# granne/granne

Measured on AMD Instinct MI355X. Metric: queries/sec (recall@10 alongside), 10M x 100-d angular, batch=1024, higher is better.
Workload: dtype f32; 1 GPU; C2 (BASELINE.json configs[1]): 10000000 x 100-d f32 angular, i.i.d. uniform components, batch=1024, ef_search=50, k=10; n_elements=10000000, dim=100, batch=1024, ef_search=50, k=10

## Files before the change

granne_amd/_lib.py:

```python
import ctypes as C
import os

from . import build as _build

F32, I8, F16 = 0, 1, 2
UNUSED = 0xFFFFFFFF
BUILD_ALL = 0xFFFFFFFFFFFFFFFF

OK = 0
ERR_INVALID, ERR_HIP, ERR_NO_DEVICE, ERR_OVERFLOW, ERR_IO = -1, -2, -3, -4, -5

OPT_VISITED_SLOTS, OPT_FORCE_SLOW, OPT_SLOW_SLOTS, OPT_SLOW_BLOCKS, OPT_OVERFLOW_SLOTS = 1, 2, 3, 4, 5
OPT_VISITED16, OPT_VISITED16_LG, OPT_LAST_WALKER, OPT_SEARCH_DEPTH, OPT_INLINE_TAILS, OPT_SEEN_MIN = 6, 7, 8, 9, 10, 11
OPT_SKETCH = 12
OPT_COALESCE, OPT_COALESCE_MAX, OPT_COALESCE_WAIT_US, OPT_COALESCED_LAUNCHES, OPT_COALESCED_QUERIES = 13, 14, 15, 16, 17
OPT_LAST_COMPACT_ROWS = 18
OPT_LAST_SPLIT_TAIL = 19
OPT_LAST_SCAN = 20
OPT_FORCE_GENERAL = 21
(SCAN_NONE, SCAN_RING, SCAN_I8, SCAN_I8_CHUNKED, SCAN_B16_7_4, SCAN_B16_13_2, SCAN_B16_16_1, SCAN_B16_CHUNKED, SCAN_F32_52_4,
 SCAN_F32_100_2, SCAN_F32_128_1) = range(11)
EXACT_TOPK_KMAX = 1024
EXACT_TOPK_CAP = 4096
PF_MAX_STAGES = 8
# ... 54 lines not shown
    "granne_hip_index_create": (i32, [C.POINTER(vp), vp, u64, u32, i32, u32, vp, vp, vp, i32]),
    "granne_hip_index_create_csr": (i32, [C.POINTER(vp), vp, u64, u32, i32, u32, vp, vp, vp, i32]),
    "granne_hip_index_create_device": (i32, [C.POINTER(vp), vp, u64, u32, i32, u32, vp, vp, vp, i32, vp]),
    "granne_hip_index_destroy": (None, [vp]),
    "granne_hip_index_len": (u64, [vp]),
    "granne_hip_index_num_elements": (u64, [vp]),
    "granne_hip_index_num_layers": (u32, [vp]),
    "granne_hip_index_layer_len": (u64, [vp, u32]),
    "granne_hip_index_dim": (u32, [vp]),
    "granne_hip_index_dtype": (i32, [vp]),
    "granne_hip_index_device": (i32, [vp]),
    "granne_hip_index_hbm_bytes": (u64, [vp]),
    "granne_hip_index_get_neighbors": (i32, [vp, u64, u32, vp, u32, C.POINTER(u32)]),
    "granne_hip_index_get_element": (i32, [vp, u64, vp]),
    "granne_hip_index_get_sketch": (i32, [vp, u64, u64, vp]),
    "granne_hip_search_batch": (i32, [vp, vp, u32, u32, u32, vp, vp, vp, vp]),
    "granne_hip_search_batch_device": (i32, [vp, vp, u32, u32, u32, vp, vp, vp, vp, vp, vp]),
    "granne_hip_search_batches_device": (i32, [vp, u32, vp, u32, u32, u32, vp, vp, vp, vp, vp, vp]),
    "granne_hip_search_begin_device": (i32, [vp, vp, u32, u32, u32, vp, vp, vp, vp, vp, vp, C.POINTER(u64)]),
    "granne_hip_search_end_device": (i32, [vp, u64, vp]),
    "granne_hip_device_malloc": (i32, [C.POINTER(vp), u64, i32]),
    "granne_hip_device_free": (i32, [vp, i32]),
    "granne_hip_copy_to_device": (i32, [vp, vp, u64, i32, vp]),
    "granne_hip_copy_to_host": (i32, [vp, vp, u64, i32, vp]),
    "granne_hip_stream_create": (i32, [C.POINTER(vp), i32]),
    "granne_hip_stream_destroy": (i32, [vp, i32]),
    "granne_hip_stream_synchronize": (i32, [vp, i32]),
    "granne_hip_event_create": (i32, [vp]),
    "granne_hip_event_destroy": (None, [vp]),
    "granne_hip_event_elapsed_ms": (i32, [vp, vp, vp]),
# ... 171 lines not shown
```

granne_amd/csrc/granne_hip.hip:

```cpp
#include <hip/hip_runtime.h>

#include <atomic>
#include <chrono>
#include <cstdarg>
#include <cstdio>
#include <cstdlib>
#include <cstring>
#include <memory>
#include <mutex>
#include <string>
#include <type_traits>
#include <vector>

#include "../../include/granne_hip.h"
#include "search_kernel.h"
#include "walk_fast.h"
#include "slow_kernel.h"
#include "util_kernels.h"
#include "brute_force.h"
#include "exact_topk.h"
#include "combiner.h"
#include "dev_mem.h"

using namespace granne_hip;
// ... 339 lines not shown
    const size_t bytes = (size_t)n * SKETCH_LINE;
    if (!ix->d_sketch) {
        size_t free_b = 0, total_b = 0;
        if (hipMemGetInfo(&free_b, &total_b) != hipSuccess) {
            (void)hipGetLastError();
            return GRANNE_HIP_OK;
        }
        if ((uint64_t)free_b < (uint64_t)bytes + total_b / 32u) return GRANNE_HIP_OK;
        if (ix->d_sketch.alloc(bytes) != hipSuccess) {
            (void)hipGetLastError();
            return GRANNE_HIP_OK;
        }
        ix->hbm_bytes += bytes;
    }
    hipLaunchKernelGGL(row_sketch_kernel, dim3(grid_for(n, 256)), dim3(256), 0, s, ix->d_elements.as<uint8_t>(), n, ix->row_stride, ix->dim,
                       ix->d_sketch.as<uint8_t>());
    HIP_TRY(hipGetLastError());
    return GRANNE_HIP_OK;
}

static int finish_layers(granne_hip_index* ix, hipStream_t s) {
    std::vector<LayerDev> h(ix->layers.size());
    ix->max_dev_width = 32;
    {
        int r = make_inline_tails(ix, s);
        if (r == 0) r = make_scan_norms(ix, s);
        if (r == 0) r = make_row_sketch(ix, s);
        if (r) return r;
    }
    DevBuf found_buf;
    std::vector<uint32_t> found(h.size(), 0u);
// ... 214 lines not shown
    *out_count = n;
    for (uint32_t i = 0; i < n && i < cap && out_ids; ++i) out_ids[i] = row[i];
    return GRANNE_HIP_OK;
}

extern "C" int granne_hip_index_get_element(const granne_hip_index* ix, uint64_t idx, void* out) {
    if (!ix || !out) return fail(GRANNE_HIP_ERR_INVALID, "null argument");
    if (idx >= ix->n_elements) return fail(GRANNE_HIP_ERR_INVALID, "element index out of range");
    if (ix->se) return se_rows_to_host(*ix->se, idx, 1, 1, (float*)out);
    DeviceGuard g(ix->device);
    HIP_TRY(hipMemcpy(out, ix->d_elements.as<uint8_t>() + idx * ix->row_stride, (size_t)ix->dim * elem_size(ix->dtype),
                      hipMemcpyDeviceToHost));
    return GRANNE_HIP_OK;
}

extern "C" int granne_hip_index_get_sketch(const granne_hip_index* ix, uint64_t first, uint64_t count, void* out) {
    if (!ix || (!out && count)) return fail(GRANNE_HIP_ERR_INVALID, "null argument");
    GRANNE_HIP_COMPACT_UNSUPPORTED(ix, "get_sketch");
    if (!ix->d_sketch) return fail(GRANNE_HIP_ERR_INVALID, "the index holds no row sketches");
    if (first > ix->n_elements || count > ix->n_elements - first) return fail(GRANNE_HIP_ERR_INVALID, "rows out of range");
    if (count == 0) return GRANNE_HIP_OK;
    DeviceGuard g(ix->device);
    HIP_TRY(hipMemcpy(out, ix->d_sketch.as<uint8_t>() + first * SKETCH_LINE, (size_t)count * SKETCH_LINE, hipMemcpyDeviceToHost));
    return GRANNE_HIP_OK;
}

extern "C" int granne_hip_index_set_option(granne_hip_index* ix, int option, uint64_t value) {
    if (!ix) return fail(GRANNE_HIP_ERR_INVALID, "index is null");
    switch (option) {
    case GRANNE_HIP_OPT_VISITED_SLOTS:
        {
            const uint64_t odd = value ? value >> __builtin_ctzll(value) : 1;
            if (value != 0 && (value < 256 || value > 32768 || (odd != 1 && odd != 3)))
                return fail(GRANNE_HIP_ERR_INVALID, "visited slots must be 0, 2^k or 3 * 2^k in [256, 32768]");
        }
// ... 387 lines not shown
    const int vmode = T.opt_visited16 ? (int)T.opt_visited16 : knobs().visited;
    const bool none = vmode == 4 || vmode == 0;
    const bool longest = walk_list_is_long((int)P.S, wide) || wide;
    uint32_t walk_lds;
    if (fast && !trail && ((none && !T.opt_visited_slots) || longest)) {
        const uint32_t touch_max = knobs().touch_max >= 0 ? (uint32_t)knobs().touch_max : 256u;
        const bool touch_shape = P.S == 1 && !wide && !streamed && !(i8 && T.stage_row_bytes != 128);
        P.v16 = (touch_shape && nq <= touch_max) ? 4 : 3;
        const uint64_t seen_min = knobs().seen_min >= 0 ? (uint64_t)knobs().seen_min : T.opt_seen_min;
        if (P.S <= 4 && !wide && !i8 && nq >= seen_min) P.v16 = 5;
        P.cr = P.v16 == 5 && !i8 && sketch_dim_ok(T.dim) && T.d_sketch != nullptr && knobs().compact_rows != 0;
        P.split = P.cr && !wide;
        walk_lds = fast_lds_bytes(i8, streamed, T.dim, T.stage_row_bytes, P.S, 0u, P.v16 == 5, wide);
        const uint32_t least = lds_query_bytes(T.stage_row_bytes) + 64u * 8u;
        if (walk_lds < least) walk_lds = least;
    } else {
        uint32_t want = T.opt_visited_slots ? (uint32_t)T.opt_visited_slots : next_pow2(ef_walk * 64u);
        if (!T.opt_visited_slots) {
            if (want < 1024) want = 1024;
            uint32_t cap = nq >= 4096 ? 4096u : 8192u;
            if (fast && P.S >= 8) cap = 4096u;
            if (want > cap) want = cap;
        }
        P.visited_slots = want;
        P.upper_slots = want < 1024 ? want : 1024;
        if (fast) {
            walk_lds = fast_lds_bytes(i8, streamed, T.dim, T.stage_row_bytes, P.S, P.visited_slots, false, wide);
        } else {
            P.adjspec_bytes = i8 ? 0u : LDS_ADJSPEC_BYTES;
            const uint32_t fixed = lds_query_bytes(T.stage_row_bytes) + LDS_FIXED_BYTES + P.adjspec_bytes;
// ... 1171 lines not shown
```

granne_amd/csrc/search_kernel.h:

```cpp
#pragma once

#include "dist.h"
#include "wave_prims.h"
#include "sum_embeddings.h"
#include "f16.h"
#include "filter.h"

namespace granne_hip {

constexpr int DT_F32 = 0;
constexpr int DT_I8 = 1;

struct LayerDev {
    const uint32_t* adj;
    uint64_t len;
    uint32_t width;
    uint32_t flags;
    const uint8_t* adjx;
    uint32_t adjx_stride;
    uint32_t reserved;
};
constexpr uint32_t LAYER_TWIN_ROWS = 1u;

constexpr uint32_t SKETCH_LINE = 128u;
constexpr uint32_t SKETCH_META = 112u;
constexpr uint32_t SKETCH_MAX_DIM = 112u;
__host__ __device__ constexpr bool sketch_dim_ok(uint32_t dim) { return dim == 100u; }

constexpr uint32_t MAX_LAUNCH_BATCHES = 32;
struct BatchIO {
    const uint8_t* queries;
    uint64_t* out_ids;
    float* out_dists;
    uint32_t* out_counts;
    uint64_t* out_stats;
};

struct SearchParams {
    const uint8_t* elements;
    uint64_t n_elements;
// ... 629 lines not shown
```

granne_amd/csrc/util_kernels.h:

```cpp
#pragma once

#include "dist.h"
#include "ordered_sum.h"
#include "search_kernel.h"

namespace granne_hip {

__device__ __forceinline__ float sketch_ceil_sqrt(double S) {
    const double T = S * (1.0 + 0x1p-40);
    if (!(T <= (double)3.4028234663852886e38 * (double)3.4028234663852886e38)) return __builtin_inff();
    float f = (float)__builtin_sqrt(T);
    while ((double)f * (double)f < T) f = __uint_as_float(__float_as_uint(f) + 1u);
    while (f > 0.0f) {
        const float g = __uint_as_float(__float_as_uint(f) - 1u);
        if ((double)g * (double)g < T) break;
        f = g;
    }
    return f;
}

__global__ void row_sketch_kernel(const uint8_t* __restrict__ elements, uint64_t n, uint32_t row_stride, uint32_t dim,
                                  uint8_t* __restrict__ out) {
    for (uint64_t row = (uint64_t)blockIdx.x * blockDim.x + threadIdx.x; row < n; row += (uint64_t)gridDim.x * blockDim.x) {
        const float* x = reinterpret_cast<const float*>(elements + row * row_stride);
        uint32_t* o = reinterpret_cast<uint32_t*>(out + row * SKETCH_LINE);
        float m = 0.0f;
        bool finite = true;
        for (uint32_t i = 0; i < dim; ++i) {
            const float a = __builtin_fabsf(x[i]);
            finite = finite && a <= 3.4028234663852886e38f;
            m = a > m ? a : m;
        }
        const float s = finite ? (float)((double)m / 127.0) : 0.0f;
        double se = 0.0, sc = 0.0, sx = 0.0;
        for (uint32_t j = 0; j < SKETCH_META / 4u; ++j) {
            uint32_t w = 0;
            for (uint32_t t = 0; t < 4u; ++t) {
// ... 2 lines not shown
                const double xd = (double)x[i];
                double c = 0.0;
                if (s > 0.0f) {
                    c = __builtin_rint(xd / (double)s);
                    c = c < -127.0 ? -127.0 : (c > 127.0 ? 127.0 : c);
                }
                const double pc = (double)s * c, e = xd - pc;
                se = se + e * e;
                sc = sc + pc * pc;
                sx = sx + xd * xd;
                w |= ((uint32_t)(int32_t)c & 0xFFu) << (8u * t);
            }
            o[j] = w;
        }
        const float inf = __builtin_inff();
        o[SKETCH_META / 4u + 0u] = __float_as_uint(s);
        o[SKETCH_META / 4u + 1u] = __float_as_uint(finite ? sketch_ceil_sqrt(se) : inf);
        o[SKETCH_META / 4u + 2u] = __float_as_uint(finite ? sketch_ceil_sqrt(sc) : inf);
        o[SKETCH_META / 4u + 3u] = __float_as_uint(finite ? sketch_ceil_sqrt(sx) : inf);
    }
}

__global__ void relayout_rows_kernel(const uint8_t* __restrict__ src, uint8_t* __restrict__ dst, uint64_t n,
                                     uint32_t src_bytes, uint32_t dst_bytes) {
    const uint32_t units = dst_bytes >> 4;
    uint64_t total = n * units;
    for (uint64_t t = (uint64_t)blockIdx.x * blockDim.x + threadIdx.x; t < total;
         t += (uint64_t)gridDim.x * blockDim.x) {
        uint64_t row = t / units;
        uint32_t u = (uint32_t)(t - row * units);
        const uint8_t* s = src + row * src_bytes + (uint64_t)u * 16;
        uint32_t avail = (u * 16 < src_bytes) ? min(16u, src_bytes - u * 16) : 0u;
        uint32_t w[4] = {0, 0, 0, 0};
        uint8_t* wb = reinterpret_cast<uint8_t*>(w);
// ... 385 lines not shown
```

granne_amd/csrc/walk_fast.h:

```cpp
#pragma once

#include <type_traits>

#include "slow_kernel.h"

namespace granne_hip {

#ifndef GRANNE_HIP_PHASE_TIMERS
#define GRANNE_HIP_PHASE_TIMERS 0
#endif
#if GRANNE_HIP_PHASE_TIMERS
constexpr uint32_t PHASE_SLOTS = 48, PHASE_QUERIES = 4096;
__device__ uint64_t g_phase[PHASE_QUERIES * PHASE_SLOTS];
#define PT_MARK(i)                                                                   \
    do {                                                                             \
        asm volatile("" ::: "memory");                                               \
        __builtin_amdgcn_sched_barrier(0);                                           \
        const uint64_t now_ = __builtin_amdgcn_s_memtime();                          \
        const uint64_t dt_ = now_ - pt_last;                                         \
        if (pt_bottom) pt_b[i] += dt_; else pt_u[i] += dt_;                          \
        pt_last = now_;                                                              \
        __builtin_amdgcn_sched_barrier(0);                                           \
        asm volatile("" ::: "memory");                                               \
    } while (0)
// ... 14 lines not shown
#define PT_COUNT() do {} while (0)
#define PT_PIN(v) do {} while (0)
#define PT_ADD(i, n) do {} while (0)
#endif

__device__ __forceinline__ uint64_t wkey(float d, uint32_t id) {
    return ((uint64_t)__float_as_uint(d) << 32) | ((uint64_t)id << 1);
}
__device__ __forceinline__ uint32_t wkey_hi(uint64_t k) { return (uint32_t)(k >> 32); }
__device__ __forceinline__ uint32_t wkey_id(uint64_t k) { return ((uint32_t)k) >> 1; }
__device__ __forceinline__ float wkey_dist(uint64_t k) { return __uint_as_float((uint32_t)(k >> 32)); }
constexpr uint32_t WPOS_NONE = 0xFFFFFFFFu;
constexpr uint32_t VCACHE_SLOTS = 512;
constexpr uint32_t VCACHE_SLOTS_SEEN = 2048;
constexpr uint64_t WALK_MAX_ELEMENTS = 1ull << 31;
#ifndef GRANNE_HIP_CR_G
#define GRANNE_HIP_CR_G 8
#endif
#ifndef GRANNE_HIP_CR_WAVES
#define GRANNE_HIP_CR_WAVES 0
#endif
static_assert(GRANNE_HIP_CR_G == 8 || GRANNE_HIP_CR_G == 4, "a surviving row is held by 8 or by 4 lanes");
static_assert(GRANNE_HIP_CR_WAVES == 0 || (GRANNE_HIP_CR_WAVES >= 4 && GRANNE_HIP_CR_WAVES <= 6), "the table's value, or four to six waves per SIMD");
__host__ __device__ constexpr int cr_waves(int S) {
    return GRANNE_HIP_CR_WAVES ? GRANNE_HIP_CR_WAVES : S == 1 ? 6 : 5;
}
__host__ __device__ constexpr uint32_t fast_vcache_slots(bool seen, bool sketched, int S) {
    return seen ? ((sketched && cr_waves(S) >= 5) ? 1024u : VCACHE_SLOTS_SEEN) : VCACHE_SLOTS;
}

// ... 306 lines not shown
            } else {
#pragma unroll
                for (int u = 0; u < TU; ++u) rr.vt[u] = *reinterpret_cast<const float4*>(row + NB * 128 + u * 16);
            }
        } else {
            const uint8_t* e = p.elements + (size_t)idl * RSTRIDE + h * 64u;
#pragma unroll
            for (int b = 0; b < NBI; ++b)
#pragma unroll
                for (int k = 0; k < 4; ++k) rr.x[b * 4 + k] = *reinterpret_cast<const uint4*>(e + b * 128 + k * 16);
        }
        asm volatile("" ::: "memory");
    }

    __device__ __forceinline__ uint64_t sketch_rejects(const uint32_t nb, const bool go, RowRegs& rr) {
        if (go) {
            const uint8_t* line = p.sketch + (size_t)nb * SKETCH_LINE + h * 64u;
#pragma unroll
            for (int k = 0; k < 4; ++k) rr.v[0][k] = *reinterpret_cast<const float4*>(line + k * 16);
        }
        asm volatile("" ::: "memory");
        int ip = 0;
#pragma unroll
        for (int k = 0; k < 4; ++k) {
            const uint4 qq = *reinterpret_cast<const uint4*>(sk_qc + h * 64u + k * 16);
            ip = dot4_i8(__float_as_uint(rr.v[0][k].x), qq.x, ip);
            ip = dot4_i8(__float_as_uint(rr.v[0][k].y), qq.y, ip);
            ip = dot4_i8(__float_as_uint(rr.v[0][k].z), qq.z, ip);
            ip = dot4_i8(__float_as_uint(rr.v[0][k].w), qq.w, ip);
        }
        ip += pair_swap(ip);
        static_assert(SKETCH_META == 64u + 48u, "s, R, X, N: the last 16 bytes of the odd lane's half");
        const float sx = rr.v[0][3].x, rx = rr.v[0][3].y, xx = rr.v[0][3].z, nx = rr.v[0][3].w;
        const float t = (sk_s * sx) * (float)ip;
        const float nqnx = sk_n * nx;
        const float b = (sk_r * xx + sk_n * rx) + nqnx * 0x1p-17f;
        const float U = t + ((__builtin_fabsf(t) * 0x1p-20f + b * 1.0001f) + 0x1p-20f);
        const float lb = 1.0f - U;
        const uint64_t rm = wave_ballot(go && h != 0u && nqnx < 0x1p100f && lb > __uint_as_float(theta));
        return rm | (rm >> 1);
    }

    __device__ __forceinline__ float finish_rows(RowRegs& rr) {
        float d;
        if constexpr (GEN) {
            float acc[16];
#pragma unroll
            for (int j = 0; j < 16; ++j) acc[j] = 0.0f;
// ... 89 lines not shown
            if (q != q) q = 0.0f;
            const float t = 1.0f - q;
            d = (0.0f <= t) ? t : 0.0f;
        }
        return d;
    }

    static constexpr int CG = CR ? CR : 8;
    static constexpr int CU = 8 / CG;
    static constexpr uint32_t CNG = 64u / CG;
    struct CRows {
        float4 v[NB ? NB : 1][CU];
        float4 vt[TU ? TU : 1];
    };
    __device__ __forceinline__ uint64_t* cr_slots() const { return mslot + CAP; }
    __device__ __forceinline__ void cr_issue(CRows& c, const uint64_t e, const bool act, const uint32_t ct, const uint8_t* xtails) const {
        if (act) {
            const uint8_t* row = p.elements + (size_t)(uint32_t)e * RSTRIDE;
#pragma unroll
            for (int b = 0; b < NB; ++b)
#pragma unroll
                for (int u = 0; u < CU; ++u) c.v[b][u] = *reinterpret_cast<const float4*>(row + b * 128 + (ct * CU + u) * 16u);
            const uint8_t* tp = xtails ? xtails + (uint32_t)(e >> 32) * XTAILB : row + NB * 128;
#pragma unroll
            for (int u = 0; u < TU; ++u) {
                const uint4 t = load_global_u4((gptr_u32)(tp + u * 16));
                c.vt[u] = make_float4(__uint_as_float(t.x), __uint_as_float(t.y), __uint_as_float(t.z), __uint_as_float(t.w));
            }
        }
    }
    __device__ __forceinline__ float cr_finish(const CRows& c, const uint32_t ct) const {
        typedef float f32x2 __attribute__((ext_vector_type(2)));
        f32x2 acc2[2 * CU];
#pragma unroll
        for (int j = 0; j < 2 * CU; ++j) acc2[j] = f32x2{0.0f, 0.0f};
#pragma unroll
        for (int b = 0; b < NB; ++b) {
#pragma unroll
            for (int u = 0; u < CU; ++u) {
                const float4 qq = *reinterpret_cast<const float4*>(lds_q + b * 128 + (ct * CU + u) * 16u);
                acc2[u * 2 + 0] = __builtin_elementwise_fma(f32x2{c.v[b][u].x, c.v[b][u].y}, f32x2{qq.x, qq.y}, acc2[u * 2 + 0]);
                acc2[u * 2 + 1] = __builtin_elementwise_fma(f32x2{c.v[b][u].z, c.v[b][u].w}, f32x2{qq.z, qq.w}, acc2[u * 2 + 1]);
// ... 11 lines not shown
            s = __uint_as_float((uint32_t)__builtin_amdgcn_update_dpp(0, __float_as_int(s), 0x111 , 0xf, 0xf, true) & keep);
#pragma unroll
            for (int j = 0; j < 4 * CU; ++j) s = s + acc[j];
        }
        float r = s;
#pragma unroll
        for (int u = 0; u < TU; ++u) {
            const float4 qq = *reinterpret_cast<const float4*>(lds_q + NB * 128 + u * 16);
            r = __builtin_fmaf(c.vt[u].x, qq.x, r);
            r = __builtin_fmaf(c.vt[u].y, qq.y, r);
            r = __builtin_fmaf(c.vt[u].z, qq.z, r);
            r = __builtin_fmaf(c.vt[u].w, qq.w, r);
        }
        return angular_from_dot(r);
    }
    __device__ __forceinline__ float compact_rows(const uint32_t ns, const uint32_t srank, const bool surv, const uint8_t* xtails) const {
        const uint32_t ct = lane & (uint32_t)(CG - 1), g = lane / (uint32_t)CG;
        const uint64_t* cs = cr_slots();
        float d = 0.0f;
        uint32_t base = 0;
        CRows ra;
#pragma unroll 1
        do {
            const uint32_t sa = base + g;
            const uint64_t ea = cs[sa];
            cr_issue(ra, ea, sa < ns, ct, xtails);
            asm volatile("" ::: "memory");
            const uint32_t rel = srank - base;
            const int from = (int)(((rel & (CNG - 1u)) * (uint32_t)CG + (uint32_t)(CG - 1)) * 4u);
            const float da = cr_finish(ra, ct);
            const float ba = __int_as_float(__builtin_amdgcn_ds_bpermute(from, __float_as_int(da)));
            d = (surv && rel < CNG) ? ba : d;
            base += CNG;
        } while (base < ns);
        return d;
    }

    static constexpr bool LONG = List::LONG;
    static constexpr int LONG_STEPS = CAP >= 4096u ? 7 : 6;
    static constexpr uint32_t FCAP = 63u;
    static constexpr uint32_t FIMG_KEYS = 128u;
// ... 521 lines not shown
            PT_MARK(8);
            PT_COUNT();
            uint64_t ykey = KEY_INF;
            uint32_t ypos = WPOS_NONE, yid = xid;
            for (uint32_t half = 0; half < (WIDE ? 2u : 1u); ++half) {
            if constexpr (WIDE) {
                if (half == 1u) nb = nb_hi;
            }
            const uint64_t unused = wave_ballot(nb == ID_EMPTY);
            const uint32_t nvalid = unused ? ((uint32_t)__builtin_ctzll(unused) >> 1) : 32u;
            st.n_adj += nvalid;
            [[maybe_unused]] uint64_t seenm = 0;
            [[maybe_unused]] uint64_t skipm = 0;
            [[maybe_unused]] uint32_t cr_ns = 0, cr_rank = 0;
            [[maybe_unused]] bool cr_surv = false;
            if constexpr (SEEN) {
                const bool seen = vcache[vcache_slot(nb)] == nb;
                seenm = wave_ballot(seen);
                if constexpr (GEN) {
                    const uint64_t newm = wave_ballot(!seen && nb != ID_EMPTY);
                    const uint32_t fill = newm ? readlane32(nb, (uint32_t)__builtin_ctzll(newm)) : xid;
                    issue_rows((!seen && nb != ID_EMPTY) ? nb : fill, rr);
                } else {
                    bool go = !seen && nb != ID_EMPTY;
                    if constexpr (SK) {
                        if (p.sketch && sk_on && theta < 0x7F800000u) {
                            skipm = sketch_rejects(nb, go, rr);
                            go = go && ((skipm >> lane) & 1ull) == 0ull;
                        }
                    }
                    if constexpr (CR != 0) {
                        const uint64_t sm = wave_ballot(go) & 0xAAAAAAAAAAAAAAAAull;
                        cr_ns = (uint32_t)__popcll(sm);
                        cr_rank = mbcnt64(sm);
                        cr_surv = go && h != 0u;
                        if (cr_surv) cr_slots()[cr_rank] = ((uint64_t)R << 32) | nb;
                    } else if (go) {
                        const uint8_t* tails = nullptr;
                        if constexpr (XT) {
                            if (adjx) tails = adjx + (size_t)xid * Ly.adjx_stride + 128u + R * XTAILB;
                        }
                        issue_rows(nb, rr, tails);
                    }
// ... 24 lines not shown
                if (nb != ID_EMPTY && !__builtin_amdgcn_inverse_ballot_w64(seenm)) vcache[vcache_slot(nb)] = nb;
            }
            asm volatile("" ::: "memory");
            __builtin_amdgcn_sched_barrier(0);
            PT_MARK(1);

            uint64_t fm;
            if constexpr (SEEN) fm = 0x5555555555555555ull & ~unused & ~seenm;
            else if constexpr (NOVIS) fm = 0x5555555555555555ull & ~unused;
            else fm = wave_ballot(vis.insert(nb, h == 0u && R < nvalid, p.ovf));
            PT_MARK(2);
            PT_WAIT_VM();
            PT_MARK(3);
            float d = 0.0f;
            if constexpr (CR != 0) {
                if (cr_ns) d = compact_rows(cr_ns, cr_rank, cr_surv, adjx ? adjx + (size_t)xid * Ly.adjx_stride + 128u : nullptr);
            } else {
                d = finish_rows(rr);
            }
            if constexpr (TOUCH) {
#pragma unroll
                for (int j = 0; j < NT; ++j) asm volatile("" ::"v"(touched[j]));
                if constexpr (XT) asm volatile("" ::"v"(touched_x));
                const uint32_t tid = next_nb != ID_EMPTY ? next_nb : yid;
                const uint8_t* tb = p.elements + (size_t)tid * RSTRIDE;
                const uint32_t lim = (XT && adjx) ? (uint32_t)NB * 128u : ROWB;
#pragma unroll
                for (int j = 0; j < NT; ++j) {
                    const uint32_t off = h * 128u + (uint32_t)j * 256u;
                    touched[j] = *reinterpret_cast<const uint32_t*>(tb + (off < lim ? off : lim - 4u));
                }
// ... 212 lines not shown
template <int DT, int DIM, int S, bool TRAIL = false, int V16 = 0, bool WIDE = false, int CR = 0>
__global__ __launch_bounds__(64, fast_waves_per_simd(DT, DIM, S, WIDE, V16 == 5, CR)) void fast_kernel(const SlowParams P) {
    extern __shared__ __align__(16) uint8_t smem[];
    if constexpr (CR != 0) {
        fast_walk_one<DT, DIM, S, TRAIL, V16, WIDE, CR>(P.sp, blockIdx.x, smem);
    } else if (blockIdx.x < P.sp.nq) {
        fast_walk_one<DT, DIM, S, TRAIL, V16, WIDE, CR>(P.sp, blockIdx.x, smem);
        walker_done(P);
    } else {
        tail_block<DT>(P, smem);
    }
}

__host__ __device__ inline uint32_t fast_lds_bytes(bool i8, bool gen, uint32_t dim, uint32_t row_bytes, uint32_t S, uint32_t visited_slots, bool seen = false, bool wide = false) {
    const bool lng = walk_list_is_long((int)S, wide);
    const uint32_t sk = (seen && !i8 && !gen && !wide && sketch_dim_ok(dim)) ? SKETCH_LINE : 0u;
    return fast_query_bytes(i8, gen, dim, row_bytes, S, seen) + (64u * S + (lng ? 0u : 32u)) * 8u + (lng ? 128u * 8u : 0u) + fast_vcache_slots(seen, sk != 0u, (int)S) * 4u + visited_slots * 4u + sk;
}

}
```

granne_amd/index.py:

```python
import ctypes as C
import os

import numpy as np

from ._lib import ERR_INVALID, ERR_OVERFLOW, EXACT_TOPK_CAP, F16, F32, I8, RANGE_CAP_MAX, GranneHipError, check, lib

DEFAULT_MAX_SEARCH = 200
DEFAULT_NUM_ELEMENTS = 10
RANGE_DEFAULT_STAGES = (252, 1020)

_ELEMENT_TYPES = {"angular": (F32, np.float32), "angular_int": (I8, np.int8), "angular_f16": (F16, np.float16)}
EMBEDDINGS = "embeddings"


def _p(a):
    return a.ctypes.data_as(C.c_void_p)


def normalize(rows, device=0):
    a = np.array(rows, dtype=np.float32, order="C", copy=True)
    flat = a.reshape(1, -1) if a.ndim == 1 else a
    if flat.size:
        check(lib().granne_hip_normalize_f32(_p(flat), flat.shape[0], flat.shape[1], device))
    return a
# ... 263 lines not shown
        check(lib().granne_hip_index_get_neighbors(self._h, idx, layer, _p(buf), buf.size, C.byref(n)))
        return buf[: n.value].astype(np.int64).tolist()

    def get_element(self, idx):
        out = np.empty(self.dim, self.np_dtype)
        check(lib().granne_hip_index_get_element(self._h, idx, _p(out)))
        return out

    def hbm_bytes(self):
        return int(lib().granne_hip_index_hbm_bytes(self._h))

    def get_sketch(self, first=0, count=None):
        count = len(self) - first if count is None else count
        out = np.empty((count, 128), np.uint8)
        if lib().granne_hip_index_get_sketch(self._h, first, count, _p(out)) != 0:
            return None
        return out

    def reorder(self):
        order = np.empty(len(self), np.uint64)
        check(lib().granne_hip_index_reorder(self._h, _p(order)))
        return order

    def reorder_by_keys(self, keys):
        k = np.ascontiguousarray(keys, dtype=np.uint64)
        if k.shape != (len(self),):
            raise ValueError("need one key per element")
        order = np.empty(len(self), np.uint64)
        check(lib().granne_hip_index_reorder_by_keys(self._h, _p(k), _p(order)))
        return order
# ... 492 lines not shown
```

include/granne.hpp:

```cpp
#pragma once

#include <algorithm>
#include <cmath>
#include <cstdint>
#include <cstring>
#include <memory>
#include <stdexcept>
#include <string>
#include <utility>
#include <vector>

#include <type_traits>

#include "granne_hip.h"

namespace granne {

inline void check(int rc) {
    if (rc != GRANNE_HIP_OK) throw std::runtime_error(std::string("granne_hip: ") + granne_hip_last_error());
}

struct f16 {
    uint16_t bits;
};
// ... 441 lines not shown
        uint64_t n = 0;
        check(granne_hip_index_encode(h_.get(), &p, &n));
        std::vector<uint8_t> out(static_cast<const uint8_t*>(p), static_cast<const uint8_t*>(p) + n);
        granne_hip_bytes_free(p);
        return out;
    }
    void set_inline_tails(bool keep) { check(granne_hip_index_set_option(h_.get(), GRANNE_HIP_OPT_INLINE_TAILS, keep ? 1 : 0)); }
    void set_seen_min(uint64_t walks) { check(granne_hip_index_set_option(h_.get(), GRANNE_HIP_OPT_SEEN_MIN, walks)); }
    void set_coalesce(bool on) { check(granne_hip_index_set_option(h_.get(), GRANNE_HIP_OPT_COALESCE, on ? 1 : 0)); }
    bool coalesce() const { return get_option(GRANNE_HIP_OPT_COALESCE) != 0; }
    void set_coalesce_max(uint64_t queries) { check(granne_hip_index_set_option(h_.get(), GRANNE_HIP_OPT_COALESCE_MAX, queries)); }
    void set_coalesce_wait_us(uint64_t us) { check(granne_hip_index_set_option(h_.get(), GRANNE_HIP_OPT_COALESCE_WAIT_US, us)); }
    uint64_t coalesced_launches() const { return get_option(GRANNE_HIP_OPT_COALESCED_LAUNCHES); }
    uint64_t coalesced_queries() const { return get_option(GRANNE_HIP_OPT_COALESCED_QUERIES); }
    bool last_compact_rows() const { return get_option(GRANNE_HIP_OPT_LAST_COMPACT_ROWS) != 0; }
    bool last_split_tail() const { return get_option(GRANNE_HIP_OPT_LAST_SPLIT_TAIL) != 0; }
    struct LastScan {
        unsigned form, ranges, prime_ranges, kk;
        bool primed;
    };
    LastScan last_scan() const {
        const uint64_t w = get_option(GRANNE_HIP_OPT_LAST_SCAN);
        return {GRANNE_HIP_LAST_SCAN_FORM(w), GRANNE_HIP_LAST_SCAN_RANGES(w), GRANNE_HIP_LAST_SCAN_PRIME_RANGES(w),
                GRANNE_HIP_LAST_SCAN_KK(w), GRANNE_HIP_LAST_SCAN_PRIMED(w) != 0};
    }
    uint64_t get_option(int option) const {
        uint64_t v = 0;
        check(granne_hip_index_get_option(h_.get(), option, &v));
        return v;
    }
// ... 449 lines not shown
```

include/granne_hip.h:

```cpp
#ifndef GRANNE_HIP_H
#define GRANNE_HIP_H

#include <stddef.h>
#include <stdint.h>

#ifdef __cplusplus
extern "C" {
#endif

#define GRANNE_HIP_ABI_VERSION 3

enum { GRANNE_HIP_F32 = 0, GRANNE_HIP_I8 = 1, GRANNE_HIP_F16 = 2 };

enum {
    GRANNE_HIP_OK = 0,
    GRANNE_HIP_ERR_INVALID = -1,
    GRANNE_HIP_ERR_HIP = -2,
    GRANNE_HIP_ERR_NO_DEVICE = -3,
    GRANNE_HIP_ERR_OVERFLOW = -4,
    GRANNE_HIP_ERR_IO = -5
};

#define GRANNE_HIP_UNUSED 0xFFFFFFFFu

// ... 20 lines not shown

void granne_hip_index_destroy(granne_hip_index* index);

uint64_t granne_hip_index_len(const granne_hip_index* index);
uint64_t granne_hip_index_num_elements(const granne_hip_index* index);
uint32_t granne_hip_index_num_layers(const granne_hip_index* index);
uint64_t granne_hip_index_layer_len(const granne_hip_index* index, uint32_t layer);
uint32_t granne_hip_index_dim(const granne_hip_index* index);
int granne_hip_index_dtype(const granne_hip_index* index);
int granne_hip_index_device(const granne_hip_index* index);
uint64_t granne_hip_index_hbm_bytes(const granne_hip_index* index);
int granne_hip_index_get_neighbors(const granne_hip_index* index, uint64_t node, uint32_t layer,
                                   uint32_t* out_ids, uint32_t cap, uint32_t* out_count);
int granne_hip_index_get_element(const granne_hip_index* index, uint64_t idx, void* out);
int granne_hip_index_get_sketch(const granne_hip_index* index, uint64_t first, uint64_t count, void* out);

int granne_hip_search_batch(const granne_hip_index* index, const void* queries, uint32_t nq,
                            uint32_t max_search, uint32_t num_neighbors, uint64_t* out_ids,
                            float* out_dists, uint32_t* out_counts, uint64_t* out_stats);

int granne_hip_search_batch_device(const granne_hip_index* index, const void* d_queries, uint32_t nq,
                                   uint32_t max_search, uint32_t num_neighbors, uint64_t* d_out_ids,
                                   float* d_out_dists, uint32_t* d_out_counts, uint64_t* d_out_stats,
                                   uint32_t* d_status, void* stream);

int granne_hip_search_batches_device(const granne_hip_index* index, uint32_t n_batches,
                                     const void* const* d_queries, uint32_t nq, uint32_t max_search,
                                     uint32_t num_neighbors, uint64_t* const* d_out_ids,
                                     float* const* d_out_dists, uint32_t* const* d_out_counts,
                                     uint64_t* const* d_out_stats, uint32_t* d_status, void* stream);
// ... 454 lines not shown
```

rust/granne-hip/src/gpu.rs:

```rust
use crate::{angular, angular_int, Index};
use std::marker::PhantomData;
use std::os::raw::{c_char, c_int, c_void};

#[repr(C)] pub struct granne_hip_index { _private: [u8; 0] }
#[repr(C)] pub struct granne_hip_builder { _private: [u8; 0] }
#[repr(C)] pub struct granne_hip_sharded { _private: [u8; 0] }
#[repr(C)] pub struct granne_hip_sum_embeddings { _private: [u8; 0] }
#[repr(C)] pub struct granne_hip_rw_builder { _private: [u8; 0] }

pub const GRANNE_HIP_F32: c_int = 0;
pub const GRANNE_HIP_I8: c_int = 1;
pub const GRANNE_HIP_F16: c_int = 2;
pub const GRANNE_HIP_BUILD_ALL: u64 = u64::MAX;

#[repr(C)]
pub struct granne_hip_build_config {
    pub layer_multiplier: f32,
    pub expected_num_elements: u64,
    pub num_neighbors: u32,
    pub max_search: u32,
    pub reinsert_elements: c_int,
    pub show_progress: c_int,
    pub batch_max: u32,
    pub batch_div: u32,
// ... 22 lines not shown
    fn granne_hip_index_load_on_device(out: *mut *mut granne_hip_index, index_bytes: *const c_void, index_len: u64,
        elements_bytes: *const c_void, elements_len: u64, dtype: c_int, device_id: c_int, staging_bytes: u64,
        out_info: *mut u64) -> c_int;
    fn granne_hip_index_load_files_on_device(out: *mut *mut granne_hip_index, index_path: *const c_char,
        elements_path: *const c_char, dtype: c_int, device_id: c_int, staging_bytes: u64, out_info: *mut u64) -> c_int;
    fn granne_hip_index_destroy(index: *mut granne_hip_index);
    fn granne_hip_index_len(index: *const granne_hip_index) -> u64;
    fn granne_hip_index_num_elements(index: *const granne_hip_index) -> u64;
    fn granne_hip_index_num_layers(index: *const granne_hip_index) -> u32;
    fn granne_hip_index_layer_len(index: *const granne_hip_index, layer: u32) -> u64;
    fn granne_hip_index_dim(index: *const granne_hip_index) -> u32;
    fn granne_hip_index_get_neighbors(index: *const granne_hip_index, node: u64, layer: u32,
        out_ids: *mut u32, cap: u32, out_count: *mut u32) -> c_int;
    fn granne_hip_index_get_element(index: *const granne_hip_index, idx: u64, out: *mut c_void) -> c_int;
    fn granne_hip_index_get_sketch(index: *const granne_hip_index, first: u64, count: u64, out: *mut c_void) -> c_int;
    fn granne_hip_search(index: *const granne_hip_index, query: *const c_void, max_search: u32,
        num_neighbors: u32, out_ids: *mut u64, out_dists: *mut f32, out_count: *mut u32) -> c_int;
    fn granne_hip_search_batch(index: *const granne_hip_index, queries: *const c_void, nq: u32,
        max_search: u32, num_neighbors: u32, out_ids: *mut u64, out_dists: *mut f32,
        out_counts: *mut u32, out_stats: *mut u64) -> c_int;
    fn granne_hip_refine_device(refine_index: *const granne_hip_index, d_queries: *const c_void, nq: u32,
        d_cand_ids: *const u64, d_cand_counts: *const u32, m: u32, k: u32, d_out_ids: *mut u64,
        d_out_dists: *mut f32, d_out_counts: *mut u32, d_refine_status: *mut u32, stream: *mut c_void) -> c_int;
    fn granne_hip_search_refined_batch_device(walk_index: *const granne_hip_index,
        refine_index: *const granne_hip_index, d_walk_queries: *const c_void, d_refine_queries: *const c_void,
        nq: u32, max_search: u32, refine_from: u32, k: u32, d_out_ids: *mut u64, d_out_dists: *mut f32,
        d_out_counts: *mut u32, d_out_stats: *mut u64, d_status: *mut u32, d_refine_status: *mut u32,
        stream: *mut c_void) -> c_int;
    fn granne_hip_search_refined_batch(walk_index: *const granne_hip_index, refine_index: *const granne_hip_index,
        walk_queries: *const c_void, refine_queries: *const c_void, nq: u32, max_search: u32, refine_from: u32,
// ... 1121 lines not shown
```

Measured before the change: 16.20 million queries/s.

## Carry row tails in device sketch lines and reuse them via LDS in compacted walk

```diff
diff --git a/granne_amd/_lib.py b/granne_amd/_lib.py
--- a/granne_amd/_lib.py
+++ b/granne_amd/_lib.py
@@ -92,6 +92,7 @@
     "granne_hip_index_get_neighbors": (i32, [vp, u64, u32, vp, u32, C.POINTER(u32)]),
     "granne_hip_index_get_element": (i32, [vp, u64, vp]),
     "granne_hip_index_get_sketch": (i32, [vp, u64, u64, vp]),
+    "granne_hip_index_get_sketch_raw": (i32, [vp, u64, u64, vp]),
     "granne_hip_search_batch": (i32, [vp, vp, u32, u32, u32, vp, vp, vp, vp]),
     "granne_hip_search_batch_device": (i32, [vp, vp, u32, u32, u32, vp, vp, vp, vp, vp, vp]),
     "granne_hip_search_batches_device": (i32, [vp, u32, vp, u32, u32, u32, vp, vp, vp, vp, vp, vp]),
diff --git a/granne_amd/csrc/granne_hip.hip b/granne_amd/csrc/granne_hip.hip
--- a/granne_amd/csrc/granne_hip.hip
+++ b/granne_amd/csrc/granne_hip.hip
@@ -377,7 +377,7 @@
         ix->hbm_bytes += bytes;
     }
     hipLaunchKernelGGL(row_sketch_kernel, dim3(grid_for(n, 256)), dim3(256), 0, s, ix->d_elements.as<uint8_t>(), n, ix->row_stride, ix->dim,
-                       ix->d_sketch.as<uint8_t>());
+                       ix->d_sketch.as<uint8_t>(), 0u);
     HIP_TRY(hipGetLastError());
     return GRANNE_HIP_OK;
 }
@@ -622,11 +622,34 @@
     return GRANNE_HIP_OK;
 }
 
-extern "C" int granne_hip_index_get_sketch(const granne_hip_index* ix, uint64_t first, uint64_t count, void* out) {
+static int sketch_rows_check(const granne_hip_index* ix, uint64_t first, uint64_t count, const void* out) {
     if (!ix || (!out && count)) return fail(GRANNE_HIP_ERR_INVALID, "null argument");
-    GRANNE_HIP_COMPACT_UNSUPPORTED(ix, "get_sketch");
     if (!ix->d_sketch) return fail(GRANNE_HIP_ERR_INVALID, "the index holds no row sketches");
     if (first > ix->n_elements || count > ix->n_elements - first) return fail(GRANNE_HIP_ERR_INVALID, "rows out of range");
+    return GRANNE_HIP_OK;
+}
+
+extern "C" int granne_hip_index_get_sketch(const granne_hip_index* ix, uint64_t first, uint64_t count, void* out) {
+    GRANNE_HIP_COMPACT_UNSUPPORTED(ix, "get_sketch");
+    if (int r = sketch_rows_check(ix, first, count, out)) return r;
+    if (count == 0) return GRANNE_HIP_OK;
+    DeviceGuard g(ix->device);
+    const uint64_t step = count < (1ull << 20) ? count : (1ull << 20);
+    DevBuf tmp;
+    HIP_TRY(tmp.alloc((size_t)step * SKETCH_LINE));
+    for (uint64_t done = 0; done < count; done += step) {
+        const uint64_t m = count - done < step ? count - done : step;
+        hipLaunchKernelGGL(row_sketch_kernel, dim3(grid_for(m, 256)), dim3(256), 0, 0,
+                           ix->d_elements.as<uint8_t>() + (first + done) * ix->row_stride, m, ix->row_stride, ix->dim, tmp.as<uint8_t>(), 1u);
+        HIP_TRY(hipGetLastError());
+        HIP_TRY(hipMemcpy((uint8_t*)out + done * SKETCH_LINE, tmp.get(), (size_t)m * SKETCH_LINE, hipMemcpyDeviceToHost));
+    }
+    return GRANNE_HIP_OK;
+}
+
+extern "C" int granne_hip_index_get_sketch_raw(const granne_hip_index* ix, uint64_t first, uint64_t count, void* out) {
+    GRANNE_HIP_COMPACT_UNSUPPORTED(ix, "get_sketch_raw");
+    if (int r = sketch_rows_check(ix, first, count, out)) return r;
     if (count == 0) return GRANNE_HIP_OK;
     DeviceGuard g(ix->device);
     HIP_TRY(hipMemcpy(out, ix->d_sketch.as<uint8_t>() + first * SKETCH_LINE, (size_t)count * SKETCH_LINE, hipMemcpyDeviceToHost));
@@ -1044,6 +1067,10 @@
         walk_lds = fast_lds_bytes(i8, streamed, T.dim, T.stage_row_bytes, P.S, 0u, P.v16 == 5, wide);
         const uint32_t least = lds_query_bytes(T.stage_row_bytes) + 64u * 8u;
         if (walk_lds < least) walk_lds = least;
+        if (P.cr && !cr_walks_fit(walk_lds, (uint32_t)cr_waves((int)P.S))) {
+            fail(GRANNE_HIP_ERR_INVALID, "the compacted walkers' LDS no longer places cr_waves walks per SIMD");
+            return P;
+        }
     } else {
         uint32_t want = T.opt_visited_slots ? (uint32_t)T.opt_visited_slots : next_pow2(ef_walk * 64u);
         if (!T.opt_visited_slots) {
diff --git a/granne_amd/csrc/search_kernel.h b/granne_amd/csrc/search_kernel.h
--- a/granne_amd/csrc/search_kernel.h
+++ b/granne_amd/csrc/search_kernel.h
@@ -24,6 +24,9 @@
 
 constexpr uint32_t SKETCH_LINE = 128u;
 constexpr uint32_t SKETCH_META = 112u;
+constexpr uint32_t SKETCH_DEV_TAIL = 100u;
+constexpr uint32_t SKETCH_DEV_META = 116u;
+constexpr float SKETCH_NORM_FACTOR = 1.0f + 0x1p-20f;
 constexpr uint32_t SKETCH_MAX_DIM = 112u;
 __host__ __device__ constexpr bool sketch_dim_ok(uint32_t dim) { return dim == 100u; }
 
diff --git a/granne_amd/csrc/util_kernels.h b/granne_amd/csrc/util_kernels.h
--- a/granne_amd/csrc/util_kernels.h
+++ b/granne_amd/csrc/util_kernels.h
@@ -20,7 +20,7 @@
 }
 
 __global__ void row_sketch_kernel(const uint8_t* __restrict__ elements, uint64_t n, uint32_t row_stride, uint32_t dim,
-                                  uint8_t* __restrict__ out) {
+                                  uint8_t* __restrict__ out, uint32_t canonical) {
     for (uint64_t row = (uint64_t)blockIdx.x * blockDim.x + threadIdx.x; row < n; row += (uint64_t)gridDim.x * blockDim.x) {
         const float* x = reinterpret_cast<const float*>(elements + row * row_stride);
         uint32_t* o = reinterpret_cast<uint32_t*>(out + row * SKETCH_LINE);
@@ -53,10 +53,15 @@
             o[j] = w;
         }
         const float inf = __builtin_inff();
-        o[SKETCH_META / 4u + 0u] = __float_as_uint(s);
-        o[SKETCH_META / 4u + 1u] = __float_as_uint(finite ? sketch_ceil_sqrt(se) : inf);
-        o[SKETCH_META / 4u + 2u] = __float_as_uint(finite ? sketch_ceil_sqrt(sc) : inf);
-        o[SKETCH_META / 4u + 3u] = __float_as_uint(finite ? sketch_ceil_sqrt(sx) : inf);
+        const uint32_t meta = (canonical ? SKETCH_META : SKETCH_DEV_META) / 4u;
+        if (!canonical) {
+            const uint32_t* xw = reinterpret_cast<const uint32_t*>(x) + (dim - 4u);
+            for (uint32_t t = 0; t < 4u; ++t) o[SKETCH_DEV_TAIL / 4u + t] = xw[t];
+        }
+        o[meta + 0u] = __float_as_uint(s);
+        o[meta + 1u] = __float_as_uint(finite ? sketch_ceil_sqrt(se) : inf);
+        o[meta + 2u] = __float_as_uint(finite ? sketch_ceil_sqrt(sc) : inf);
+        if (canonical) o[meta + 3u] = __float_as_uint(finite ? sketch_ceil_sqrt(sx) : inf);
     }
 }
 
diff --git a/granne_amd/csrc/walk_fast.h b/granne_amd/csrc/walk_fast.h
--- a/granne_amd/csrc/walk_fast.h
+++ b/granne_amd/csrc/walk_fast.h
@@ -52,6 +52,11 @@
 constexpr uint32_t VCACHE_SLOTS = 512;
 constexpr uint32_t VCACHE_SLOTS_SEEN = 2048;
 constexpr uint64_t WALK_MAX_ELEMENTS = 1ull << 31;
+constexpr uint32_t CR_TAILS_BYTES = 32u * 16u;
+constexpr uint32_t LDS_CU_BYTES = 160u * 1024u, LDS_ALLOC_UNIT = 1280u;
+__host__ __device__ constexpr bool cr_walks_fit(uint32_t walk_lds, uint32_t waves_per_simd) {
+    return (walk_lds + LDS_ALLOC_UNIT - 1u) / LDS_ALLOC_UNIT * LDS_ALLOC_UNIT * 4u * waves_per_simd <= LDS_CU_BYTES;
+}
 #ifndef GRANNE_HIP_CR_G
 #define GRANNE_HIP_CR_G 8
 #endif
@@ -388,24 +393,30 @@
     }
 
     __device__ __forceinline__ uint64_t sketch_rejects(const uint32_t nb, const bool go, RowRegs& rr) {
+        float4 own[4];
+        float4(&sv)[4] = CR != 0 ? own : rr.v[0];
         if (go) {
             const uint8_t* line = p.sketch + (size_t)nb * SKETCH_LINE + h * 64u;
 #pragma unroll
-            for (int k = 0; k < 4; ++k) rr.v[0][k] = *reinterpret_cast<const float4*>(line + k * 16);
+            for (int k = 0; k < 4; ++k) sv[k] = *reinterpret_cast<const float4*>(line + k * 16);
         }
         asm volatile("" ::: "memory");
         int ip = 0;
 #pragma unroll
         for (int k = 0; k < 4; ++k) {
             const uint4 qq = *reinterpret_cast<const uint4*>(sk_qc + h * 64u + k * 16);
-            ip = dot4_i8(__float_as_uint(rr.v[0][k].x), qq.x, ip);
-            ip = dot4_i8(__float_as_uint(rr.v[0][k].y), qq.y, ip);
-            ip = dot4_i8(__float_as_uint(rr.v[0][k].z), qq.z, ip);
-            ip = dot4_i8(__float_as_uint(rr.v[0][k].w), qq.w, ip);
+            ip = dot4_i8(__float_as_uint(sv[k].x), qq.x, ip);
+            ip = dot4_i8(__float_as_uint(sv[k].y), qq.y, ip);
+            ip = dot4_i8(__float_as_uint(sv[k].z), qq.z, ip);
+            ip = dot4_i8(__float_as_uint(sv[k].w), qq.w, ip);
+        }
+        if constexpr (CR != 0) {
+            if (go && h != 0u) cr_tails()[R] = make_float4(sv[2].y, sv[2].z, sv[2].w, sv[3].x);
         }
         ip += pair_swap(ip);
-        static_assert(SKETCH_META == 64u + 48u, "s, R, X, N: the last 16 bytes of the odd lane's half");
-        const float sx = rr.v[0][3].x, rx = rr.v[0][3].y, xx = rr.v[0][3].z, nx = rr.v[0][3].w;
+        static_assert(SKETCH_DEV_META == 64u + 48u + 4u && SKETCH_DEV_TAIL == 64u + 32u + 4u, "the tail, then s, R, X: the odd lane's last 28 bytes");
+        const float sx = sv[3].y, rx = sv[3].z, xx = sv[3].w;
+        const float nx = (xx + rx) * SKETCH_NORM_FACTOR;
         const float t = (sk_s * sx) * (float)ip;
         const float nqnx = sk_n * nx;
         const float b = (sk_r * xx + sk_n * rx) + nqnx * 0x1p-17f;
@@ -525,18 +536,24 @@
         float4 vt[TU ? TU : 1];
     };
     __device__ __forceinline__ uint64_t* cr_slots() const { return mslot + CAP; }
-    __device__ __forceinline__ void cr_issue(CRows& c, const uint64_t e, const bool act, const uint32_t ct, const uint8_t* xtails) const {
+    __device__ __forceinline__ float4* cr_tails() const { return reinterpret_cast<float4*>(sk_qc + SKETCH_LINE); }
+    static_assert(TU == 1 || CR == 0, "the kept sketch line carries one 16-byte tail");
+    __device__ __forceinline__ void cr_issue(CRows& c, const uint64_t e, const bool act, const uint32_t ct, const uint8_t* xtails,
+                                             const bool lds_tails = false) const {
         if (act) {
+            if (lds_tails) c.vt[0] = cr_tails()[(uint32_t)(e >> 32)];
             const uint8_t* row = p.elements + (size_t)(uint32_t)e * RSTRIDE;
 #pragma unroll
             for (int b = 0; b < NB; ++b)
 #pragma unroll
                 for (int u = 0; u < CU; ++u) c.v[b][u] = *reinterpret_cast<const float4*>(row + b * 128 + (ct * CU + u) * 16u);
-            const uint8_t* tp = xtails ? xtails + (uint32_t)(e >> 32) * XTAILB : row + NB * 128;
-#pragma unroll
-            for (int u = 0; u < TU; ++u) {
-                const uint4 t = load_global_u4((gptr_u32)(tp + u * 16));
-                c.vt[u] = make_float4(__uint_as_float(t.x), __uint_as_float(t.y), __uint_as_float(t.z), __uint_as_float(t.w));
+            if (!lds_tails) {
+                const uint8_t* tp = xtails ? xtails + (uint32_t)(e >> 32) * XTAILB : row + NB * 128;
+#pragma unroll
+                for (int u = 0; u < TU; ++u) {
+                    const uint4 t = load_global_u4((gptr_u32)(tp + u * 16));
+                    c.vt[u] = make_float4(__uint_as_float(t.x), __uint_as_float(t.y), __uint_as_float(t.z), __uint_as_float(t.w));
+                }
             }
         }
     }
@@ -578,7 +595,7 @@
         }
         return angular_from_dot(r);
     }
-    __device__ __forceinline__ float compact_rows(const uint32_t ns, const uint32_t srank, const bool surv, const uint8_t* xtails) const {
+    __device__ __forceinline__ float compact_rows(const uint32_t ns, const uint32_t srank, const bool surv, const uint8_t* xtails, const bool lds_tails) const {
         const uint32_t ct = lane & (uint32_t)(CG - 1), g = lane / (uint32_t)CG;
         const uint64_t* cs = cr_slots();
         float d = 0.0f;
@@ -588,7 +605,7 @@
         do {
             const uint32_t sa = base + g;
             const uint64_t ea = cs[sa];
-            cr_issue(ra, ea, sa < ns, ct, xtails);
+            cr_issue(ra, ea, sa < ns, ct, xtails, lds_tails);
             asm volatile("" ::: "memory");
             const uint32_t rel = srank - base;
             const int from = (int)(((rel & (CNG - 1u)) * (uint32_t)CG + (uint32_t)(CG - 1)) * 4u);
@@ -1140,6 +1157,7 @@
             [[maybe_unused]] uint64_t skipm = 0;
             [[maybe_unused]] uint32_t cr_ns = 0, cr_rank = 0;
             [[maybe_unused]] bool cr_surv = false;
+            [[maybe_unused]] bool cr_lds = false;
             if constexpr (SEEN) {
                 const bool seen = vcache[vcache_slot(nb)] == nb;
                 seenm = wave_ballot(seen);
@@ -1153,6 +1171,7 @@
                         if (p.sketch && sk_on && theta < 0x7F800000u) {
                             skipm = sketch_rejects(nb, go, rr);
                             go = go && ((skipm >> lane) & 1ull) == 0ull;
+                            if constexpr (CR != 0) cr_lds = true;
                         }
                     }
                     if constexpr (CR != 0) {
@@ -1207,7 +1226,7 @@
             PT_MARK(3);
             float d = 0.0f;
             if constexpr (CR != 0) {
-                if (cr_ns) d = compact_rows(cr_ns, cr_rank, cr_surv, adjx ? adjx + (size_t)xid * Ly.adjx_stride + 128u : nullptr);
+                if (cr_ns) d = compact_rows(cr_ns, cr_rank, cr_surv, adjx ? adjx + (size_t)xid * Ly.adjx_stride + 128u : nullptr, cr_lds);
             } else {
                 d = finish_rows(rr);
             }
@@ -1450,7 +1469,7 @@
 
 __host__ __device__ inline uint32_t fast_lds_bytes(bool i8, bool gen, uint32_t dim, uint32_t row_bytes, uint32_t S, uint32_t visited_slots, bool seen = false, bool wide = false) {
     const bool lng = walk_list_is_long((int)S, wide);
-    const uint32_t sk = (seen && !i8 && !gen && !wide && sketch_dim_ok(dim)) ? SKETCH_LINE : 0u;
+    const uint32_t sk = (seen && !i8 && !gen && !wide && sketch_dim_ok(dim)) ? SKETCH_LINE + CR_TAILS_BYTES : 0u;
     return fast_query_bytes(i8, gen, dim, row_bytes, S, seen) + (64u * S + (lng ? 0u : 32u)) * 8u + (lng ? 128u * 8u : 0u) + fast_vcache_slots(seen, sk != 0u, (int)S) * 4u + visited_slots * 4u + sk;
 }
 
diff --git a/granne_amd/index.py b/granne_amd/index.py
--- a/granne_amd/index.py
+++ b/granne_amd/index.py
@@ -301,6 +301,13 @@
         count = len(self) - first if count is None else count
         out = np.empty((count, 128), np.uint8)
         if lib().granne_hip_index_get_sketch(self._h, first, count, _p(out)) != 0:
+            return None
+        return out
+
+    def get_sketch_raw(self, first=0, count=None):
+        count = len(self) - first if count is None else count
+        out = np.empty((count, 128), np.uint8)
+        if lib().granne_hip_index_get_sketch_raw(self._h, first, count, _p(out)) != 0:
             return None
         return out
 
diff --git a/include/granne.hpp b/include/granne.hpp
--- a/include/granne.hpp
+++ b/include/granne.hpp
@@ -479,6 +479,16 @@
     uint64_t coalesced_launches() const { return get_option(GRANNE_HIP_OPT_COALESCED_LAUNCHES); }
     uint64_t coalesced_queries() const { return get_option(GRANNE_HIP_OPT_COALESCED_QUERIES); }
     bool last_compact_rows() const { return get_option(GRANNE_HIP_OPT_LAST_COMPACT_ROWS) != 0; }
+    std::vector<uint8_t> get_sketch(size_t first, size_t count) const {
+        std::vector<uint8_t> out(count * 128);
+        check(granne_hip_index_get_sketch(h_.get(), first, count, out.data()));
+        return out;
+    }
+    std::vector<uint8_t> get_sketch_raw(size_t first, size_t count) const {
+        std::vector<uint8_t> out(count * 128);
+        check(granne_hip_index_get_sketch_raw(h_.get(), first, count, out.data()));
+        return out;
+    }
     bool last_split_tail() const { return get_option(GRANNE_HIP_OPT_LAST_SPLIT_TAIL) != 0; }
     struct LastScan {
         unsigned form, ranges, prime_ranges, kk;
diff --git a/include/granne_hip.h b/include/granne_hip.h
--- a/include/granne_hip.h
+++ b/include/granne_hip.h
@@ -58,6 +58,7 @@
                                    uint32_t* out_ids, uint32_t cap, uint32_t* out_count);
 int granne_hip_index_get_element(const granne_hip_index* index, uint64_t idx, void* out);
 int granne_hip_index_get_sketch(const granne_hip_index* index, uint64_t first, uint64_t count, void* out);
+int granne_hip_index_get_sketch_raw(const granne_hip_index* index, uint64_t first, uint64_t count, void* out);
 
 int granne_hip_search_batch(const granne_hip_index* index, const void* queries, uint32_t nq,
                             uint32_t max_search, uint32_t num_neighbors, uint64_t* out_ids,
diff --git a/rust/granne-hip/src/gpu.rs b/rust/granne-hip/src/gpu.rs
--- a/rust/granne-hip/src/gpu.rs
+++ b/rust/granne-hip/src/gpu.rs
@@ -60,6 +60,7 @@
         out_ids: *mut u32, cap: u32, out_count: *mut u32) -> c_int;
     fn granne_hip_index_get_element(index: *const granne_hip_index, idx: u64, out: *mut c_void) -> c_int;
     fn granne_hip_index_get_sketch(index: *const granne_hip_index, first: u64, count: u64, out: *mut c_void) -> c_int;
+    fn granne_hip_index_get_sketch_raw(index: *const granne_hip_index, first: u64, count: u64, out: *mut c_void) -> c_int;
     fn granne_hip_search(index: *const granne_hip_index, query: *const c_void, max_search: u32,
         num_neighbors: u32, out_ids: *mut u64, out_dists: *mut f32, out_count: *mut u32) -> c_int;
     fn granne_hip_search_batch(index: *const granne_hip_index, queries: *const c_void, nq: u32,
```

After: 16.78 million queries/s (median of 6 runs). 3.6% higher.
